# nlesc-dirac/sagecal

Measured on NVIDIA H100. Metric: baseline_visibilities_per_sec_predict_jacobian, higher is better.
Workload: dtype f64

## Files before the change

### sagecal_b200/csrc/internal.cuh

```cuda
#pragma once
#include <cuda_runtime.h>
#include <stdint.h>
#include <stdio.h>
#include <stdlib.h>

#define DB_CHECK(call)                                                                          \
  do {                                                                                          \
    cudaError_t err__ = (call);                                                                 \
    if (err__ != cudaSuccess) {                                                                 \
      fprintf(stderr, "dirac_b200: CUDA error %s at %s:%d: %s\n", cudaGetErrorName(err__),      \
              __FILE__, __LINE__, cudaGetErrorString(err__));                                   \
      exit(1);          \
    }                                                                                           \
  } while (0)


#define TILE_P 8
#define TILE_Q 32
#define TILE_THREADS (TILE_P * TILE_Q)

struct TileDesc {
  short pb, qb;
};

// ... 203 lines not shown
  int N, Nbase;
  int t_begin, t_end, tslice;
};

struct StreamAllArgs {
  const double2 *coh;
  const double2 *x;
  const unsigned char *flag;
  const double *pp;
  const double *pk;
  const ClusterDesc *clus;
  const int *chunk_poff;
  const short2 *blpq;
  double2 *out;
  double2 *E0, *E1, *E2;
  double *partials, *cost;
  unsigned int *counter;
  long long R;
  int N, Nbase, tilesz, M;
  int out_mode, cost_mode;
  double inv_nu;
  int partial;
  long long row0;
  long long w_lo, w_hi;
};

struct GramArgs {
  const double2 *coh;
  const unsigned char *flag;
  const TileDesc *tiles;
// ... 8 lines not shown
  const double *T;
  const double *pblk;
  const int *list;
  const int *tix;
  const int *poff;
  double *JTJ;
  long long stride;
  double *Hst;
  const double *mu_dev;
  double mu;
  int lower;
  int N, Nbase;
};

enum { DB_OPT_CP_ROWS = 0, DB_OPT_LINE_DIRECT = 1, DB_OPT_OS_CONSISTENT = 2,
       DB_OPT_RTR_NU_UNJOINED = 3, DB_OPT_ADMM_LM = 4, DB_OPT_COUNT = 8 };
int db_opt(int id);
int db_sm_count();
static inline int db_cp_max_slices(int Nbase, int tilesz) {
  const int nbg = (Nbase + 255) / 256;
  int nsl = (db_sm_count() + nbg - 1) / nbg;
  if ((tilesz + 31) / 32 > nsl) nsl = (tilesz + 31) / 32;
  return nsl;
}

extern "C" {
void db_launch_coh_to_planar(const double2 *src, double2 *dst, long long r0, int nr, int M,
                             long long R, cudaStream_t st);
void db_launch_coh_from_planar(const double2 *src, double2 *dst, long long r0, int nr, int M,
                               long long R, cudaStream_t st);
void db_launch_vis_to_planar(const double2 *src, double2 *dst, long long R, cudaStream_t st);
// ... 21 lines not shown
                            cudaStream_t st);
void db_launch_chol_factor_batched(const double *A, int n, const double *mu, double *ws,
                                   long long ws_stride, int *info, int nb, cudaStream_t st);
void db_launch_chol_solve(const double *A, int n, double mu, const double *b, double *x, double *ws,
                          int *info, cudaStream_t st);
int db_bigtri_available(int n);
size_t db_bigtri_ws_doubles(int n);
void db_launch_bigtri_solve(const double *L, int ld, int n, const double *b, double *x, double *ws,
                            unsigned epoch, int invert, cudaStream_t st);
int db_stream_all_nblocks(int Nbase, int tilesz);
void db_launch_predict_tma(const StreamAllArgs *a, cudaStream_t st);
void db_launch_cost_window_tma(const StreamAllArgs *a, cudaStream_t st);
int db_band_nblocks(int Nbase, int tilesz, int nchan);
void db_launch_band_tma(const StreamAllArgs *a, int nchan, cudaStream_t st);
void db_launch_band_tma(const StreamAllArgs *a, int nchan, cudaStream_t st);
void db_launch_line_setup_tma(const StreamAllArgs *a, cudaStream_t st);
void db_line_setup_shape_reset();
void db_line_setup_shape(int *shape);
}
```

### sagecal_b200/csrc/kernels_line.cu

```cuda
#include "internal.cuh"

__device__ __forceinline__ void grid_reduce_sum_l(double v, double *partials, double *out,
                                                  unsigned int *counter) {
  __shared__ double wsum[32];
  __shared__ bool is_last;
  v = warp_sum(v);
  const int lane = threadIdx.x & 31, w = threadIdx.x >> 5;
  if (lane == 0) wsum[w] = v;
  __syncthreads();
  const unsigned int nblocks = gridDim.x * gridDim.y;
  const unsigned int bid = blockIdx.x + gridDim.x * blockIdx.y;
  if (threadIdx.x == 0) {
    double s = 0.0;
    const int nw = (blockDim.x + 31) >> 5;
    for (int i = 0; i < nw; i++) s += wsum[i];
    partials[bid] = s;
    __threadfence();
    is_last = (atomicAdd(counter, 1u) == nblocks - 1);
  }
  __syncthreads();
  if (is_last) {
    double s = 0.0;
    for (unsigned int i = threadIdx.x; i < nblocks; i += blockDim.x)
      s += ((volatile double *)partials)[i];
// ... 21 lines not shown
       i += (long long)gridDim.x * blockDim.x) {
    const double2 e0 = E0[i], e1 = E1[i], e2 = E2[i];
    const double ex = (e0.x - alpha * e1.x) - a2 * e2.x;
    const double ey = (e0.y - alpha * e1.y) - a2 * e2.y;
    if (mode == 1) {
      s = fma(ex, ex, s);
      s = fma(ey, ey, s);
    } else {
      s += log(1.0 + ex * ex * inv_nu);
      s += log(1.0 + ey * ey * inv_nu);
    }
  }
  grid_reduce_sum_l(s, partials, out, counter);
}

__global__ void __launch_bounds__(256)
k_line_poly(const double2 *__restrict__ E0, const double2 *__restrict__ E1,
            const double2 *__restrict__ E2, long long n4, double *partials, double *out,
            unsigned int *counter) {
  double c[5] = {0.0, 0.0, 0.0, 0.0, 0.0};
  for (long long i = (long long)blockIdx.x * blockDim.x + threadIdx.x; i < n4;
       i += (long long)gridDim.x * blockDim.x) {
    const double2 e0 = E0[i], e1 = E1[i], e2 = E2[i];
    c[0] = fma(e0.x, e0.x, fma(e0.y, e0.y, c[0]));
    c[1] = fma(e0.x, e1.x, fma(e0.y, e1.y, c[1]));
    c[2] = fma(e1.x, e1.x, fma(e1.y, e1.y, c[2]));
    c[2] = fma(-2.0 * e0.x, e2.x, fma(-2.0 * e0.y, e2.y, c[2]));
    c[3] = fma(e1.x, e2.x, fma(e1.y, e2.y, c[3]));
    c[4] = fma(e2.x, e2.x, fma(e2.y, e2.y, c[4]));
  }
  __shared__ double ws[5][8];
  __shared__ bool is_last;
  const int lane = threadIdx.x & 31, w = threadIdx.x >> 5;
#pragma unroll
  for (int j = 0; j < 5; j++) {
    const double v = warp_sum(c[j]);
    if (lane == 0) ws[j][w] = v;
  }
  __syncthreads();
  if (threadIdx.x < 5) {
    double s = 0.0;
    for (int i = 0; i < 8; i++) s += ws[threadIdx.x][i];
    partials[(size_t)blockIdx.x * 5 + threadIdx.x] = s;
  }
  __threadfence();
  __syncthreads();
  if (threadIdx.x == 0) is_last = (atomicAdd(counter, 1u) == gridDim.x - 1);
  __syncthreads();
  if (is_last && threadIdx.x < 5) {
    double s = 0.0;
    for (unsigned int b = 0; b < gridDim.x; b++)
      s += ((volatile double *)partials)[(size_t)b * 5 + threadIdx.x];
    if (threadIdx.x == 1) s *= -2.0;
    if (threadIdx.x == 3) s *= 2.0;
    out[threadIdx.x] = s;
    if (threadIdx.x == 0) *counter = 0;
  }
}

__global__ void __launch_bounds__(256)
k_line_residual(const double2 *__restrict__ E0, const double2 *__restrict__ E1,
                const double2 *__restrict__ E2, double2 *__restrict__ res, long long n4,
                double alpha) {
  const double a2 = alpha * alpha;
  for (long long i = (long long)blockIdx.x * blockDim.x + threadIdx.x; i < n4;
       i += (long long)gridDim.x * blockDim.x) {
    const double2 e0 = E0[i], e1 = E1[i], e2 = E2[i];
    res[i] = make_double2((e0.x - alpha * e1.x) - a2 * e2.x, (e0.y - alpha * e1.y) - a2 * e2.y);
  }
}

__global__ void __launch_bounds__(256)
// ... 83 lines not shown
void db_launch_axpby(const double2 *x, double2 *y, long long n4, double a, double b,
                     cudaStream_t st) {
  k_axpby<<<592, 256, 0, st>>>(x, y, n4, a, b);
}
void db_launch_cluster_rowmap(const double2 *coh_k, const double2 *in, const double2 *in2,
                               double2 *out, const unsigned char *flag, const double *pp,
                               const int *chunk_poff, int nchunk, const short2 *blpq, long long R,
                               int Nbase, int sign, double beta, cudaStream_t st) {
  k_cluster_rowmap<<<592, 256, 0, st>>>(coh_k, in, in2, out, flag, pp, chunk_poff, nchunk, blpq, R,
                                        Nbase, sign, beta);
}
void db_launch_line_poly(const double2 *E0, const double2 *E1, const double2 *E2, long long n4,
                         double *partials, double *out, unsigned int *counter, cudaStream_t st) {
  k_line_poly<<<192, 256, 0, st>>>(E0, E1, E2, n4, partials, out, counter);
}
void db_launch_line_residual(const double2 *E0, const double2 *E1, const double2 *E2, double2 *res,
                             long long n4, double alpha, cudaStream_t st) {
  k_line_residual<<<LINE_GRID, 256, 0, st>>>(E0, E1, E2, res, n4, alpha);
}
}
```

### sagecal_b200/csrc/kernels_tma.cu

```cuda
#include "internal.cuh"
#include "tma.cuh"

template <int MODE, int TB, int NST, int WARPS>
__global__ void __launch_bounds__(WARPS * 32)
k_stream_all(StreamAllArgs a) {
  extern __shared__ __align__(128) unsigned char smem_raw[];
  constexpr int STAGE_ELEMS = TB * 4 * 32;
  constexpr int NACC = (MODE == 1) ? 3 : 1;
  constexpr size_t RING_BYTES = (size_t)WARPS * NST * STAGE_ELEMS * 16;
  constexpr size_t COMB_BYTES = (size_t)(WARPS - 1) * NACC * STAGE_ELEMS * 16;
  constexpr size_t DATA_BYTES = RING_BYTES > COMB_BYTES ? RING_BYTES : COMB_BYTES;
  double2 *ring = reinterpret_cast<double2 *>(smem_raw);
  unsigned long long *bars = reinterpret_cast<unsigned long long *>(smem_raw + DATA_BYTES);
  const int w = threadIdx.x >> 5, lane = threadIdx.x & 31;
  double2 *my_stage = ring + (size_t)w * NST * STAGE_ELEMS;
  unsigned long long *my_bar = bars + w * NST;
  if (lane == 0) {
#pragma unroll
    for (int s = 0; s < NST; s++) mbar_init(&my_bar[s], 1);
    mbar_fence_init();
  }
  __syncwarp();

  const int nbg = (a.Nbase + 31) >> 5;
// ... 96 lines not shown
  if (w > 0) {
#pragma unroll
    for (int i = 0; i < TB; i++)
#pragma unroll
      for (int c = 0; c < 4; c++) {
        double2 *dst = comb + ((size_t)(w - 1) * NACC * TB * 4 + (i * 4 + c)) * 32 + lane;
        dst[0] = V0[i][c];
        if (MODE == 1) {
          dst[(size_t)TB * 4 * 32] = V1[i][c];
          dst[(size_t)2 * TB * 4 * 32] = V2[i][c];
        }
      }
  }
  __syncthreads();
  double cost = 0.0;
  if (w == 0 && valid) {
    for (int ww = 1; ww < WARPS; ww++)
#pragma unroll
      for (int i = 0; i < TB; i++)
#pragma unroll
        for (int c = 0; c < 4; c++) {
          const double2 *src = comb + ((size_t)(ww - 1) * NACC * TB * 4 + (i * 4 + c)) * 32 + lane;
          V0[i][c] = cadd(V0[i][c], src[0]);
          if (MODE == 1) {
            V1[i][c] = cadd(V1[i][c], src[(size_t)TB * 4 * 32]);
            V2[i][c] = cadd(V2[i][c], src[(size_t)2 * TB * 4 * 32]);
          }
        }
#pragma unroll
    for (int i = 0; i < TB; i++) {
// ... 9 lines not shown
          if (MODE != 1) {
            double2 xv = z;
            if (a.out_mode == 1 || a.cost_mode) xv = ld_stream(a.x + ix);
            const double2 e = csub(xv, m);
            if (a.out_mode == 1) st_stream(a.out + ix, e);
            if (a.out_mode == 2) st_stream(a.out + ix, m);
            if (a.cost_mode == 1) {
              cost = fma(e.x, e.x, cost);
              cost = fma(e.y, e.y, cost);
            } else if (a.cost_mode == 2) {
              cost += log(1.0 + e.x * e.x * a.inv_nu);
              cost += log(1.0 + e.y * e.y * a.inv_nu);
            }
          } else {
            const double2 xv = ld_stream(a.x + ix);
            st_stream(a.E0 + ix, a.partial ? m : csub(xv, m));
            st_stream(a.E1 + ix, fl ? z : V1[i][c]);
            st_stream(a.E2 + ix, fl ? z : V2[i][c]);
          }
        }
      }
    }
  }
  if (MODE != 1 && a.cost_mode) {
    __shared__ bool is_last;
    cost = warp_sum(cost);
    if (threadIdx.x == 0) {
      a.partials[blockIdx.x] = cost;
      __threadfence();
      is_last = (atomicAdd(a.counter, 1u) == gridDim.x - 1);
    }
    __syncthreads();
    if (is_last && w == 0) {
      double s = 0.0;
      for (unsigned int i = lane; i < gridDim.x; i += 32) s += ((volatile double *)a.partials)[i];
      s = warp_sum(s);
      if (lane == 0) {
        *a.cost = s;
        *a.counter = 0;
      }
    }
  }
}

static int g_line_shape[3] = {-1, -1, -1};

template <int MODE, int TB, int NST, int WARPS>
static void launch_cfg(const StreamAllArgs *a, cudaStream_t st) {
  if (MODE == 1) {
    g_line_shape[0] = TB;
    g_line_shape[1] = NST;
    g_line_shape[2] = WARPS;
  }
  const int nbg = (a->Nbase + 31) / 32, ntb = (a->tilesz + TB - 1) / TB;
  const unsigned grid = (unsigned)((long long)nbg * ntb);
  constexpr int NACC = (MODE == 1) ? 3 : 1;
  const size_t ring = (size_t)WARPS * NST * TB * 4 * 32 * 16;
  const size_t comb = (size_t)(WARPS - 1) * NACC * TB * 4 * 32 * 16;
  const size_t smem = (ring > comb ? ring : comb) + WARPS * NST * 8;
  static bool configured = false;
  if (!configured) {
    DB_CHECK(cudaFuncSetAttribute(k_stream_all<MODE, TB, NST, WARPS>,
                                  cudaFuncAttributeMaxDynamicSharedMemorySize, (int)smem));
    configured = true;
  }
  k_stream_all<MODE, TB, NST, WARPS><<<grid, WARPS * 32, smem, st>>>(*a);
}

extern "C" {
int db_stream_all_nblocks(int Nbase, int tilesz) {
  const int nbg = (Nbase + 31) / 32;
  return (int)((long long)nbg * tilesz);
}
void db_launch_predict_tma(const StreamAllArgs *a, cudaStream_t st) {
  launch_cfg<0, 2, 2, 3>(a, st);
}
void db_launch_cost_window_tma(const StreamAllArgs *a, cudaStream_t st) {
  launch_cfg<2, 2, 2, 3>(a, st);
}
void db_launch_line_setup_tma(const StreamAllArgs *a, cudaStream_t st) {
  const long long items = (long long)((a->Nbase + 31) / 32) * a->tilesz;
  if (items >= 64ll * db_sm_count()) launch_cfg<1, 1, 4, 1>(a, st);
  else launch_cfg<1, 1, 2, 3>(a, st);
}
void db_line_setup_shape_reset() { g_line_shape[0] = g_line_shape[1] = g_line_shape[2] = -1; }
void db_line_setup_shape(int *shape) {
  for (int i = 0; i < 3; i++) shape[i] = g_line_shape[i];
}
}
```

### sagecal_b200/csrc/lbfgs.cu

```cuda
#include <float.h>
#include <math.h>
#include <string.h>
#include <vector>

#include "problem.h"

extern "C" {
int db_lbfgs_direction_max_pairs(void);
void db_launch_lbfgs_direction(double *pk, const double *gk, const double *s, const double *y,
                               const double *rho, int m, int npairs, int next, cudaStream_t st);
void db_launch_lbfgs_nrm2(const double *g, int m, double *out, cudaStream_t st);
void db_launch_lbfgs_step(const double *xk, const double *pk, const double *gk, double *xk1,
                          double *sk, double *yk, int m, double alpha, cudaStream_t st);
void db_launch_lbfgs_update(const double *gk, const double *sk, double *yk, const double *xk1,
                            double *xk, int m, double *rho_slot, double *out, cudaStream_t st);
void db_launch_line_eval(const double2 *E0, const double2 *E1, const double2 *E2, long long n4,
                         double alpha, int mode, double inv_nu, double *partials, double *out,
                         unsigned int *counter, cudaStream_t st);
void db_launch_line_residual(const double2 *E0, const double2 *E1, const double2 *E2, double2 *res,
                             long long n4, double alpha, cudaStream_t st);
void db_launch_line_poly(const double2 *E0, const double2 *E1, const double2 *E2, long long n4,
                         double *partials, double *out, unsigned int *counter, cudaStream_t st);
}

struct LbfgsCtx {
  dirac_b200_problem *pr;
  int robust;
  double nu;
  int m;
  long long ncost, ngrad;
  double poly[5];
};

static void line_alloc(dirac_b200_problem *pr) {
  if (pr->E0) return;
  DevProblem &d = pr->d;
  const size_t n = (size_t)4 * d.R;
  pr->E0 = (decltype(pr->E0))db_malloc(sizeof(double2) * n * 3);
  pr->E1 = pr->E0 + n;
  pr->E2 = pr->E1 + n;
}

static void line_setup(LbfgsCtx *c, const double *xk, const double *pk) {
  dirac_b200_problem *pr = c->pr;
  DevProblem &d = pr->d;
  line_alloc(pr);
  StreamAllArgs s;
  memset(&s, 0, sizeof(s));
  s.coh = d.coh; s.x = d.x; s.flag = d.flag; s.pp = xk; s.pk = pk; s.clus = d.clus;
  s.chunk_poff = d.chunk_poff; s.blpq = d.blpq; s.E0 = pr->E0; s.E1 = pr->E1; s.E2 = pr->E2;
  s.R = d.R; s.N = d.N; s.Nbase = d.Nbase; s.tilesz = d.tilesz; s.M = d.M;
  s.partial = (pr->world > 1) ? 1 : 0;
  if (db_overlap_available(pr) && d.tilesz >= 8) {
    static cudaEvent_t ev_chunk[8], ev_done;
    static bool have_ev = false;
    if (!have_ev) {
      for (int i = 0; i < 8; i++) DB_CHECK(cudaEventCreateWithFlags(&ev_chunk[i], cudaEventDisableTiming));
      DB_CHECK(cudaEventCreateWithFlags(&ev_done, cudaEventDisableTiming));
      have_ev = true;
    }
    cudaStream_t cs = db_comm_stream();
    const int nch = 8;
    const int per = (d.tilesz + nch - 1) / nch;
    db_prof_begin(7, (double)d.R * (64.0 * d.M + 65.0 + 192.0), d.stream);
    int ci = 0;
    for (int t0 = 0; t0 < d.tilesz; t0 += per, ci++) {
      const int t1 = (t0 + per < d.tilesz) ? t0 + per : d.tilesz;
// ... 11 lines not shown
      for (int v = 0; v < 3; v++)
        for (int c = 0; c < 4; c++) {
          double2 *base = (v == 0 ? pr->E0 : v == 1 ? pr->E1 : pr->E2) + (long long)c * d.R + r0;
          seg[v * 4 + c] = reinterpret_cast<double *>(base);
          cnt[v * 4 + c] = 2 * nr;
        }
      db_allreduce_segments(pr, seg, cnt, 12, cs);
    }
    db_prof_end(d.stream);
    DB_CHECK(cudaEventRecord(ev_done, cs));
    DB_CHECK(cudaStreamWaitEvent(d.stream, ev_done, 0));
    db_launch_axpby(d.x, pr->E0, 4 * d.R, 1.0, -1.0, d.stream);
    db_count_launch(1);
  } else {
    db_prof_begin(7, (double)d.R * (64.0 * d.M + 65.0 + 192.0), d.stream);
    db_launch_line_setup_tma(&s, d.stream);
    db_prof_end(d.stream);
    db_count_launch(1);
    if (pr->world > 1) {
      db_allreduce(pr, pr->E0, 3 * 8 * d.R);
      db_launch_axpby(d.x, pr->E0, 4 * d.R, 1.0, -1.0, d.stream);
      db_count_launch(1);
    }
  }
  if (!c->robust && !db_opt(DB_OPT_LINE_DIRECT)) {
    db_launch_line_poly(pr->E0, pr->E1, pr->E2, 4 * d.R, pr->partials, d.scal + 16, d.counters,
                        d.stream);
    db_count_launch(1);
    DB_CHECK(cudaMemcpyAsync(d.h_scal + 16, d.scal + 16, 5 * sizeof(double), cudaMemcpyDeviceToHost,
                             d.stream));
    db_stream_sync(d.stream);
    for (int j = 0; j < 5; j++) c->poly[j] = d.h_scal[16 + j];
  }
}

static double line_cost(LbfgsCtx *c, double alpha) {
  dirac_b200_problem *pr = c->pr;
  DevProblem &d = pr->d;
  if (!c->robust && !db_opt(DB_OPT_LINE_DIRECT)) {
    c->ncost++;
    const double *q = c->poly;
    return q[0] + alpha * (q[1] + alpha * (q[2] + alpha * (q[3] + alpha * q[4])));
  }
  db_launch_line_eval(pr->E0, pr->E1, pr->E2, 4 * d.R, alpha, c->robust ? 2 : 1,
                      c->robust ? 1.0 / c->nu : 0.0, pr->partials, d.scal, d.counters, d.stream);
  db_count_launch(1);
  c->ncost++;
  return db_read_scalar(pr, 0);
}

static void grad_eval(LbfgsCtx *c, const double *p, double *g, bool from_line, double alpha) {
  dirac_b200_problem *pr = c->pr;
  DevProblem &d = pr->d;
  if (from_line) {
    db_launch_line_residual(pr->E0, pr->E1, pr->E2, pr->res, 4 * d.R, alpha, d.stream);
    db_count_launch(1);
  } else {
    db_predict_dev(pr, p, pr->res, 1, 0, 0.0, 0);
  }
  db_grad_dev(pr, p, g, c->robust, c->nu);
  c->ngrad++;
}

static double cubic_interp(LbfgsCtx *c, double a, double b, double *xa, double step) {
  double f0, f1, f0d, f1d, p01, p02, z0, fz0, aa, cc;
  *xa = a;
  f0 = line_cost(c, *xa);
  *xa += step;
  p01 = line_cost(c, *xa);
  *xa += -2.0 * step;
  p02 = line_cost(c, *xa);
  f0d = (p01 - p02) / (2.0 * step);
// ... 121 lines not shown
    phi_alphai1 = phi_alphai;
    ci++;
  }
  return alphak;
}

struct LbfgsTrace {
  double *alphak;
  long long *ncost;
  int *slot;
  double *gnorm;
  double *iterates;
  int niter;
};

static void lbfgs_run(dirac_b200_problem *pr, double *p, int m, int itmax, int M, int robust,
                      double nu, LbfgsTrace *tr) {
  DevProblem &d = pr->d;
  LbfgsCtx ctx;
  ctx.pr = pr;
  ctx.robust = robust;
  ctx.nu = nu;
  ctx.m = m;
  ctx.ncost = ctx.ngrad = 0;
  if (tr) tr->niter = 0;
  if (M < 1) M = 1;
  if (M > db_lbfgs_direction_max_pairs()) {
    fprintf(stderr, "dirac_b200: LBFGS memory size %d exceeds the %d pairs the two-loop recursion "
                    "can hold; the LBFGS stage is skipped\n", M, db_lbfgs_direction_max_pairs());
    return;
  }
  double *ws = (double *)db_malloc(sizeof(double) * ((size_t)m * (4 + 2 * (size_t)M) + M + 8));
  double *xk = ws, *xk1 = xk + m, *gk = xk1 + m, *pk = gk + m, *s = pk + m,
         *y = s + (size_t)m * M, *rho = y + (size_t)m * M;
  double *nrm_dev = d.scal + 24;
  double step, alphak;
  int ck, ci, cm;
  DB_CHECK(cudaMemcpyAsync(xk, p, sizeof(double) * m, cudaMemcpyHostToDevice, d.stream));
  grad_eval(&ctx, xk, gk, false, 0.0);
  db_launch_lbfgs_nrm2(gk, m, nrm_dev, d.stream);
  db_count_launch(1);
  double gradnrm = sqrt(db_read_scalar(pr, 24));
  const double STOP = 1e-17;
  if (gradnrm < STOP) {
    ck = itmax;
    step = 0.0;
  } else {
    ck = 0;
    double t = 1e-3 / gradnrm;
    if (t > 1e-6) t = 1e-6;
    step = (t > 1e-9) ? t : 1e-9;
  }
  cm = 0;
  ci = 0;
  while (ck < itmax && isnormal(gradnrm) && gradnrm > STOP) {
    const long long ncost0 = ctx.ncost;
    db_launch_lbfgs_direction(pk, gk, s, y, rho, m, ck < M ? ck : M, ci, d.stream);
    db_count_launch(1);
    line_setup(&ctx, xk, pk);
    alphak = linesearch(&ctx, 10.0, 0.1, 0.01, 9, 0.1, 0.5, step);
    if (!isnormal(alphak) || fabs(alphak) < 1e-12) break;
    double *sk = s + (size_t)cm;
    double *yk = y + (size_t)cm;
    db_launch_lbfgs_step(xk, pk, gk, xk1, sk, yk, m, alphak, d.stream);
    grad_eval(&ctx, xk1, gk, true, alphak);
    db_launch_lbfgs_update(gk, sk, yk, xk1, xk, m, rho + ci, nrm_dev, d.stream);
    db_count_launch(2);
    gradnrm = sqrt(db_read_scalar(pr, 24));
    if (tr) {
      tr->alphak[ck] = alphak;
      tr->ncost[ck] = ctx.ncost - ncost0;
      tr->slot[ck] = ci;
      tr->gnorm[ck] = gradnrm;
      DB_CHECK(cudaMemcpy(tr->iterates + (size_t)m * ck, xk, sizeof(double) * m,
                          cudaMemcpyDeviceToHost));
      tr->niter = ck + 1;
    }
    ck++;
    if (cm < (M - 1) * m) {
      cm += m;
      ci++;
    } else {
      cm = ci = 0;
    }
  }
  DB_CHECK(cudaMemcpyAsync(p, xk, sizeof(double) * m, cudaMemcpyDeviceToHost, d.stream));
  db_stream_sync(d.stream);
  db_free(ws);
}

void db_lbfgs_fit(dirac_b200_problem *pr, double *p, int m, int itmax, int M, int robust,
                  double nu) {
  lbfgs_run(pr, p, m, itmax, M, robust, nu, nullptr);
}

extern "C" void dirac_b200_line_model(dirac_b200_problem *pr, const double *xk, const double *pk,
                                      int nalpha, const double *alphas, double nu,
                                      double alpha_res, double *E, double *poly, double *costs,
                                      double *res, int *shape) {
  DevProblem &d = pr->d;
  LbfgsCtx c;
  c.pr = pr; c.robust = 0; c.nu = nu; c.m = (int)d.npar; c.ncost = c.ngrad = 0;
  double *dx = (double *)db_malloc(sizeof(double) * 2 * d.npar);
  double *dp = dx + d.npar;
  DB_CHECK(cudaMemcpyAsync(dx, xk, sizeof(double) * d.npar, cudaMemcpyHostToDevice, d.stream));
  DB_CHECK(cudaMemcpyAsync(dp, pk, sizeof(double) * d.npar, cudaMemcpyHostToDevice, d.stream));
  db_line_setup_shape_reset();
  line_setup(&c, dx, dp);
// ... 2 lines not shown
  for (int i = 0; i < nalpha; i++)
    for (int mode = 1; mode <= 2; mode++) {
      db_launch_line_eval(pr->E0, pr->E1, pr->E2, 4 * d.R, alphas[i], mode,
                          mode == 2 ? 1.0 / nu : 0.0, pr->partials, d.scal, d.counters, d.stream);
      costs[2 * i + mode - 1] = db_read_scalar(pr, 0);
    }
  db_download_vis(pr, pr->E0, E);
  db_download_vis(pr, pr->E1, E + 8 * d.R);
  db_download_vis(pr, pr->E2, E + 16 * d.R);
  db_launch_line_residual(pr->E0, pr->E1, pr->E2, pr->res, 4 * d.R, alpha_res, d.stream);
  db_download_vis(pr, pr->res, res);
  DB_CHECK(cudaGetLastError());
  db_free(dx);
}

extern "C" int dirac_b200_lbfgs_trace(dirac_b200_problem *pr, double *p, int itmax, int M, int robust,
                                      double nu, double *alphak, long long *ncost, int *slot,
                                      double *gnorm, double *iterates) {
  if ((M < 1 ? 1 : M) > db_lbfgs_direction_max_pairs()) return -1;
  LbfgsTrace tr;
  tr.alphak = alphak; tr.ncost = ncost; tr.slot = slot; tr.gnorm = gnorm; tr.iterates = iterates;
  lbfgs_run(pr, p, (int)pr->d.npar, itmax, M, robust, nu, &tr);
  return tr.niter;
}

extern "C" int dirac_b200_lbfgs_direction(int m, int Mmem, int npairs, int next, const double *g,
                                          const double *s, const double *y, const double *rho,
                                          double *pk) {
  if (m < 1 || Mmem < 1 || npairs < 0 || npairs > Mmem || next < 0 || next >= Mmem ||
      npairs > db_lbfgs_direction_max_pairs())
    return -1;
  const size_t nv = (size_t)m * (2 + 2 * (size_t)Mmem) + Mmem;
  double *w = (double *)db_malloc(sizeof(double) * nv);
  double *dg = w, *dpk = dg + m, *ds = dpk + m, *dy = ds + (size_t)m * Mmem,
         *drho = dy + (size_t)m * Mmem;
  DB_CHECK(cudaMemcpy(dg, g, sizeof(double) * m, cudaMemcpyHostToDevice));
  DB_CHECK(cudaMemcpy(ds, s, sizeof(double) * m * Mmem, cudaMemcpyHostToDevice));
// ... 48 lines not shown
```

### sagecal_b200/csrc/problem.cu

```cuda
#include <string.h>
#include <thread>
#include <vector>

#include "../../include/dirac_b200.h"
#include "internal.cuh"
#include "problem.h"

static unsigned long long g_launches = 0;
static unsigned long long g_sky_uploads = 0, g_coh_host_bytes = 0;
void db_count_sky_upload() { g_sky_uploads++; }
void db_count_coh_host_bytes(size_t bytes) { g_coh_host_bytes += bytes; }
extern "C" void dirac_b200_transfer_stats(unsigned long long *sky_uploads,
                                          unsigned long long *coh_host_bytes, int reset) {
  if (sky_uploads) *sky_uploads = g_sky_uploads;
  if (coh_host_bytes) *coh_host_bytes = g_coh_host_bytes;
  if (reset) g_sky_uploads = g_coh_host_bytes = 0;
}
void db_count_launch(int n) { g_launches += (unsigned long long)n; }
extern "C" unsigned long long dirac_b200_launch_count(void) { return g_launches; }

struct ProfRec { cudaEvent_t a, b; int kind; double bytes; };
static std::vector<ProfRec> g_prof;
static std::vector<cudaEvent_t> g_evpool;
static int g_prof_on = 0;
// ... 45 lines not shown
  if (g_have_user_stream) { *owned = 0; return g_user_stream; }
  cudaStream_t st;
  DB_CHECK(cudaStreamCreateWithFlags(&st, cudaStreamNonBlocking));
  *owned = 1;
  return st;
}

static int g_opt[DB_OPT_COUNT] = {0, 0, 0, 0, 0, 0, 0, 0};
int db_opt(int id) { return (id >= 0 && id < DB_OPT_COUNT) ? g_opt[id] : 0; }
extern "C" int dirac_b200_set_option(const char *name, int value) {
  if (!strcmp(name, "cp_rows")) { g_opt[DB_OPT_CP_ROWS] = value; return 0; }
  if (!strcmp(name, "line_direct")) { g_opt[DB_OPT_LINE_DIRECT] = value; return 0; }
  if (!strcmp(name, "os_consistent")) { g_opt[DB_OPT_OS_CONSISTENT] = value; return 0; }
  if (!strcmp(name, "rtr_nu_unjoined")) { g_opt[DB_OPT_RTR_NU_UNJOINED] = value; return 0; }
  if (!strcmp(name, "admm_lm")) { g_opt[DB_OPT_ADMM_LM] = value; return 0; }
  return -1;
}
int db_sm_count() {
  static int n[64];
  int dev = 0;
  if (cudaGetDevice(&dev) != cudaSuccess || dev < 0 || dev >= 64) return 132;
  if (!n[dev]) {
    int v = 0;
    if (cudaDeviceGetAttribute(&v, cudaDevAttrMultiProcessorCount, dev) != cudaSuccess || v <= 0) v = 132;
    n[dev] = v;
  }
  return n[dev];
}

void require_gpu() {
// ... 506 lines not shown
```

### sagecal_b200/csrc/problem.h

```cpp
#pragma once
#include <cusolverDn.h>
#include <cublas_v2.h>

#include <vector>

#include "../../include/dirac_b200.h"
#include "internal.cuh"

struct BigChol;
BigChol *db_bigchol_create(int n, int nbk, bool inv_panel, bool lookahead);
enum { BC_BLOCK = 256 };
static const bool BC_INV_PANEL = true, BC_LOOKAHEAD = true;
void db_bigchol_destroy(BigChol *bc);
void db_bigchol_bind_batch(BigChol *bc, double *A0, long long stride, int maxb);
void db_bigchol_factor_batch(BigChol *bc, int nb, int *info, int info_step, cudaStream_t st);

struct LMWork {
  bool ready;
  int n8;
  double *T;
  unsigned char *T_valid;
  double *Tsub;
  double *JTJ0, *JTJ;
  double *JTe, *JTe_new;
// ... 46 lines not shown
  double *g;
  LMWork lm;
  int own_stream;
  int rank, world;
  void (*allreduce)(void *dev, long long count, void *stream, void *user);
  void *comm_user;
  int m_global;
  int k_global0;
  double beta;
  const double *aug_y_host, *aug_bz_host, *aug_rho;
  double *aug_dev;
  double2 *pm;
  double *xb;
  double *pp_start;
  double2 *E0, *E1, *E2;
  struct RtrWork *rtr;
};

void db_stream_sync(cudaStream_t st);
void db_event_sync(cudaEvent_t ev);
void db_flag_wait(const volatile unsigned long long *flag, unsigned long long epoch,
                  cudaStream_t st);
void *db_malloc(size_t bytes);
void db_free(void *p);
void require_gpu();

class DeviceScope {
 public:
  DeviceScope();
  explicit DeviceScope(cudaStream_t borrowed);
// ... 46 lines not shown
void db_allreduce_world(dirac_b200_problem *pr, void *dev, long long count);
int db_nccl_world();
void db_allreduce_stream(dirac_b200_allreduce_fn fn, void *user, void *dev, long long count,
                         cudaStream_t st);
int db_manifold_projectback(double *Y, int n, int Mt, int Nf, int Niter, const int *cr,
                            cudaStream_t st);void db_lm_set_aug(const double *y_dev, const double *bz_dev, const double *y_host,
                   const double *bz_host, double rho);
int db_overlap_available(const dirac_b200_problem *pr);
cudaStream_t db_comm_stream();
void db_allreduce_segments(dirac_b200_problem *pr, double **ptr, const long long *count, int nseg,
                           cudaStream_t st);
extern "C" {
void db_launch_residual_cost(const double2 *x, const double2 *pm, double2 *out, long long n4,
                             int out_mode, int cost_mode, double inv_nu, double *partials,
                             double *cost, unsigned int *counter, cudaStream_t st);
void db_launch_axpby(const double2 *x, double2 *y, long long n4, double a, double b,
                     cudaStream_t st);
void db_launch_cluster_rowmap(const double2 *coh_k, const double2 *in, const double2 *in2,
                              double2 *out, const unsigned char *flag, const double *pp,
                              const int *chunk_poff, int nchunk, const short2 *blpq, long long R,
                              int Nbase, int sign, double beta, cudaStream_t st);
}

struct BandView {
  const double2 *coh, *x;
  const unsigned char *flag;
  int nc;
};
struct BandDev {
  int N, Nbase, tilesz, M, Mt, maxnc, ntile;
// ... 24 lines not shown
```

### sagecal_b200/csrc/sage.cu

```cuda
#include <math.h>
#include <string.h>
#include <thread>
#include <vector>

#include "../../include/dirac_b200.h"
#include "problem.h"

void db_lm_chunk(dirac_b200_problem *pr, int k, int ck, double *pblk_dev, double2 *r, int itmax,
                 const double *opts, int linsolv, int os, int randomize, double *info,
                 bool hidden_ready);
void db_rlm_chunk(dirac_b200_problem *pr, int k, int ck, double *pblk_dev, double2 *r, int itmax,
                  int linsolv, int os, int randomize, double nulow, double nuhigh,
                  double *robust_nu, double *info, bool hidden_ready);
bool db_cluster_needs_rowmap(const dirac_b200_problem *pr, int k);
void db_cluster_hidden(dirac_b200_problem *pr, int k, double2 *r, int sign, double beta);
void db_lbfgs_fit(dirac_b200_problem *pr, double *p, int m, int itmax, int M, int robust,
                  double nu);
void db_lbfgs_fit_minibatch(dirac_b200_problem *pr, double *p, int m, int itmax, int M, double nu);
void db_rtr_chunk(dirac_b200_problem *pr, int k, int ck, double *pblk_dev, double2 *r, int kind,
                  int itmax_a, int itmax_b, double nulow, double nuhigh, double *robust_nu,
                  double *info, bool hidden_ready, const double *aug_y, const double *aug_bz,
                  double aug_rho);
#define SM_RTR_ADMM_ 7

static bool is_robust_mode(int solver_mode) {
  return solver_mode == SM_OSLM_OSRLM_RLBFGS || solver_mode == SM_RLM_RLBFGS ||
         solver_mode == SM_RTR_OSRLM_RLBFGS || solver_mode == SM_NSD_RLBFGS ||
         solver_mode == SM_RTR_ADMM_;
}

extern "C" int dirac_b200_sagefit(dirac_b200_problem *pr, double *pp, double *x_out,
                                  int max_emiter, int max_iter, int max_lbfgs, int lbfgs_m,
// ... 168 lines not shown
    if (total_err > 0.0)
      for (int cj = 0; cj < MG; cj++) nerr[cj] *= 1.0 / total_err;
    if (randomize) weighted_iter = !weighted_iter;
  }
  if (robust) {
    if (sharded) allreduce_host(robust_nuM.data(), MG);
    double s = 0.0;
    for (int cj = 0; cj < MG; cj++) s += fabs(robust_nuM[cj]);
    robust_nu0 = s / (double)MG;
    if (robust_nu0 < nulow) robust_nu0 = nulow;
    else if (robust_nu0 > nuhigh) robust_nu0 = nuhigh;
  }
  DB_CHECK(cudaMemcpyAsync(pp, d.pp, sizeof(double) * m, cudaMemcpyDeviceToHost, d.stream));
  db_stream_sync(d.stream);

  if (max_lbfgs > 0) {
    if (robust) {
      if (lbfgs_m > 0) {
        db_lbfgs_fit(pr, pp, m, max_lbfgs, lbfgs_m, 1, robust_nu0);
      } else if (lbfgs_m < 0) {
        db_lbfgs_fit_minibatch(pr, pp, m, max_lbfgs, -lbfgs_m, robust_nu0);
      }
    } else {
      db_lbfgs_fit(pr, pp, m, max_lbfgs, lbfgs_m, 0, 0.0);
    }
  }
  DB_CHECK(cudaMemcpyAsync(d.pp, pp, sizeof(double) * m, cudaMemcpyHostToDevice, d.stream));
  db_predict_dev(pr, d.pp, pr->res, 1, 1, 0.0, 0);
  *res_1 = sqrt(db_read_scalar(pr, 0)) / (double)n;
  if (x_out) db_download_vis(pr, pr->res, x_out);
  *mean_nu = robust_nu0;
  DB_CHECK(cudaGetLastError());
  return (*res_1 > *res_0) ? -1 : 0;
}

extern "C" int sagefit_visibilities(double *u, double *v, double *w, double *x, int N, int Nbase,
                                    int tilesz, baseline_t *barr, clus_source_t *carr,
                                    double *coh, int M, int Mt, double freq0, double fdelta,
                                    double *pp, double uvmin, int Nt, int max_emiter, int max_iter,
                                    int max_lbfgs, int lbfgs_m, int gpu_threads, int linsolv,
                                    int solver_mode, double nulow, double nuhigh, int randomize,
                                    double *mean_nu, double *res_0, double *res_1) {
  (void)u; (void)v; (void)w; (void)freq0; (void)fdelta; (void)uvmin; (void)Nt; (void)gpu_threads;
// ... 19 lines not shown
SAGEFIT_ALIAS(sagefit_visibilities_dual_pt_flt)
SAGEFIT_ALIAS(sagefit_visibilities_dual_pt)
SAGEFIT_ALIAS(sagefit_visibilities_dual_pt_one_gpu)

int db_bfgsfit_dev(dirac_b200_problem *pr, double *pp, int max_lbfgs, int lbfgs_m, int solver_mode,
                   double mean_nu, double *res_0, double *res_1, bool keep_residual) {
  DevProblem &d = pr->d;
  const int m = d.N * d.Mt * 8;
  const long long n = (long long)d.Nbase * d.tilesz * 8;
  DB_CHECK(cudaMemcpyAsync(d.pp, pp, sizeof(double) * m, cudaMemcpyHostToDevice, d.stream));
  db_predict_dev(pr, d.pp, nullptr, 0, 1, 0.0, 0);
  *res_0 = sqrt(db_read_scalar(pr, 0)) / (double)n;
  if (max_lbfgs > 0) {
    int M_ = lbfgs_m > 0 ? lbfgs_m : -lbfgs_m;
    if (is_robust_mode(solver_mode)) {
      db_lbfgs_fit(pr, pp, m, max_lbfgs, M_, 1, mean_nu);
    } else {
      db_lbfgs_fit(pr, pp, m, max_lbfgs, M_, 0, 0.0);
    }
  }
  DB_CHECK(cudaMemcpyAsync(d.pp, pp, sizeof(double) * m, cudaMemcpyHostToDevice, d.stream));
  db_predict_dev(pr, d.pp, keep_residual ? pr->res : nullptr, keep_residual ? 1 : 0, 1, 0.0, 0);
  *res_1 = sqrt(db_read_scalar(pr, 0)) / (double)n;
  return (*res_1 > *res_0) ? -1 : 0;
}

extern "C" int bfgsfit_visibilities(double *u, double *v, double *w, double *x, int N, int Nbase,
                                    int tilesz, baseline_t *barr, clus_source_t *carr,
                                    double *coh, int M, int Mt, double freq0, double fdelta,
                                    double *pp, double uvmin, int Nt, int max_lbfgs, int lbfgs_m,
                                    int gpu_threads, int solver_mode, double mean_nu,
                                    double *res_0, double *res_1) {
  (void)u; (void)v; (void)w; (void)freq0; (void)fdelta; (void)uvmin; (void)Nt; (void)gpu_threads;
// ... 78 lines not shown
```

Measured before the change: 6.816 billion.

## Fold line-search polynomial into setup kernel and reuse held residuals after LBFGS

The line-setup streaming kernel now accumulates the five line-search polynomial coefficients while it writes E0/E1/E2. A small finish kernel then reduces the per-block partials, so the separate pass that re-read all three arrays is no longer needed on the single-device path. The LBFGS stage can also start from the residual already held on the device instead of re-predicting it. After LBFGS, the final cost is taken as a sum of squares over the held residual rather than a full re-predict. This cuts memory passes and predict launches in the sagefit path, at the price of extra registers in the streaming kernel and an assumption that the held residual matches the final parameters.

New measurement: 7.071 billion (median of 6 runs). +3.7%, better.

```diff
diff --git a/sagecal_b200/csrc/internal.cuh b/sagecal_b200/csrc/internal.cuh
--- a/sagecal_b200/csrc/internal.cuh
+++ b/sagecal_b200/csrc/internal.cuh
@@ -241,6 +241,7 @@
   const short2 *blpq;
   double2 *out;
   double2 *E0, *E1, *E2;
+  double *poly_part;
   double *partials, *cost;
   unsigned int *counter;
   long long R;
@@ -279,7 +280,8 @@
 };
 
 enum { DB_OPT_CP_ROWS = 0, DB_OPT_LINE_DIRECT = 1, DB_OPT_OS_CONSISTENT = 2,
-       DB_OPT_RTR_NU_UNJOINED = 3, DB_OPT_ADMM_LM = 4, DB_OPT_COUNT = 8 };
+       DB_OPT_RTR_NU_UNJOINED = 3, DB_OPT_ADMM_LM = 4, DB_OPT_SWEEP_RESIDUAL = 5,
+       DB_OPT_COUNT = 8 };
 int db_opt(int id);
 int db_sm_count();
 static inline int db_cp_max_slices(int Nbase, int tilesz) {
@@ -331,7 +333,9 @@
 int db_band_nblocks(int Nbase, int tilesz, int nchan);
 void db_launch_band_tma(const StreamAllArgs *a, int nchan, cudaStream_t st);
 void db_launch_band_tma(const StreamAllArgs *a, int nchan, cudaStream_t st);
-void db_launch_line_setup_tma(const StreamAllArgs *a, cudaStream_t st);
+unsigned db_launch_line_setup_tma(const StreamAllArgs *a, cudaStream_t st);
+void db_launch_line_poly_finish(const double *part, unsigned nparts, double *partials, double *out,
+                                unsigned int *counter, cudaStream_t st);
 void db_line_setup_shape_reset();
 void db_line_setup_shape(int *shape);
 }
diff --git a/sagecal_b200/csrc/kernels_line.cu b/sagecal_b200/csrc/kernels_line.cu
--- a/sagecal_b200/csrc/kernels_line.cu
+++ b/sagecal_b200/csrc/kernels_line.cu
@@ -59,6 +59,37 @@
   grid_reduce_sum_l(s, partials, out, counter);
 }
 
+__device__ __forceinline__ void poly_grid_reduce(const double *c, double *partials, double *out,
+                                                 unsigned int *counter) {
+  __shared__ double ws[5][8];
+  __shared__ bool is_last;
+  const int lane = threadIdx.x & 31, w = threadIdx.x >> 5;
+#pragma unroll
+  for (int j = 0; j < 5; j++) {
+    const double v = warp_sum(c[j]);
+    if (lane == 0) ws[j][w] = v;
+  }
+  __syncthreads();
+  if (threadIdx.x < 5) {
+    double s = 0.0;
+    for (int i = 0; i < 8; i++) s += ws[threadIdx.x][i];
+    partials[(size_t)blockIdx.x * 5 + threadIdx.x] = s;
+  }
+  __threadfence();
+  __syncthreads();
+  if (threadIdx.x == 0) is_last = (atomicAdd(counter, 1u) == gridDim.x - 1);
+  __syncthreads();
+  if (is_last && threadIdx.x < 5) {
+    double s = 0.0;
+    for (unsigned int b = 0; b < gridDim.x; b++)
+      s += ((volatile double *)partials)[(size_t)b * 5 + threadIdx.x];
+    if (threadIdx.x == 1) s *= -2.0;
+    if (threadIdx.x == 3) s *= 2.0;
+    out[threadIdx.x] = s;
+    if (threadIdx.x == 0) *counter = 0;
+  }
+}
+
 __global__ void __launch_bounds__(256)
 k_line_poly(const double2 *__restrict__ E0, const double2 *__restrict__ E1,
             const double2 *__restrict__ E2, long long n4, double *partials, double *out,
@@ -74,33 +105,30 @@
     c[3] = fma(e1.x, e2.x, fma(e1.y, e2.y, c[3]));
     c[4] = fma(e2.x, e2.x, fma(e2.y, e2.y, c[4]));
   }
-  __shared__ double ws[5][8];
-  __shared__ bool is_last;
-  const int lane = threadIdx.x & 31, w = threadIdx.x >> 5;
-#pragma unroll
-  for (int j = 0; j < 5; j++) {
-    const double v = warp_sum(c[j]);
-    if (lane == 0) ws[j][w] = v;
-  }
-  __syncthreads();
-  if (threadIdx.x < 5) {
-    double s = 0.0;
-    for (int i = 0; i < 8; i++) s += ws[threadIdx.x][i];
-    partials[(size_t)blockIdx.x * 5 + threadIdx.x] = s;
-  }
-  __threadfence();
-  __syncthreads();
-  if (threadIdx.x == 0) is_last = (atomicAdd(counter, 1u) == gridDim.x - 1);
-  __syncthreads();
-  if (is_last && threadIdx.x < 5) {
-    double s = 0.0;
-    for (unsigned int b = 0; b < gridDim.x; b++)
-      s += ((volatile double *)partials)[(size_t)b * 5 + threadIdx.x];
-    if (threadIdx.x == 1) s *= -2.0;
-    if (threadIdx.x == 3) s *= 2.0;
-    out[threadIdx.x] = s;
-    if (threadIdx.x == 0) *counter = 0;
-  }
+  poly_grid_reduce(c, partials, out, counter);
+}
+
+__global__ void __launch_bounds__(256)
+k_line_poly_finish(const double *__restrict__ part, unsigned nparts, double *partials, double *out,
+                   unsigned int *counter) {
+  double c[5] = {0.0, 0.0, 0.0, 0.0, 0.0};
+  for (unsigned i = blockIdx.x * blockDim.x + threadIdx.x; i < nparts; i += gridDim.x * blockDim.x)
+#pragma unroll
+    for (int j = 0; j < 5; j++) c[j] += part[(size_t)j * nparts + i];
+  poly_grid_reduce(c, partials, out, counter);
+}
+
+__global__ void __launch_bounds__(256)
+k_sumsq(const double2 *__restrict__ v, long long n4, double *partials, double *out,
+        unsigned int *counter) {
+  double s = 0.0;
+  for (long long i = (long long)blockIdx.x * blockDim.x + threadIdx.x; i < n4;
+       i += (long long)gridDim.x * blockDim.x) {
+    const double2 e = v[i];
+    s = fma(e.x, e.x, s);
+    s = fma(e.y, e.y, s);
+  }
+  grid_reduce_sum_l(s, partials, out, counter);
 }
 
 __global__ void __launch_bounds__(256)
@@ -214,6 +242,14 @@
                          double *partials, double *out, unsigned int *counter, cudaStream_t st) {
   k_line_poly<<<192, 256, 0, st>>>(E0, E1, E2, n4, partials, out, counter);
 }
+void db_launch_line_poly_finish(const double *part, unsigned nparts, double *partials, double *out,
+                                unsigned int *counter, cudaStream_t st) {
+  k_line_poly_finish<<<192, 256, 0, st>>>(part, nparts, partials, out, counter);
+}
+void db_launch_sumsq(const double2 *v, long long n4, double *partials, double *out,
+                     unsigned int *counter, cudaStream_t st) {
+  k_sumsq<<<LINE_GRID, 256, 0, st>>>(v, n4, partials, out, counter);
+}
 void db_launch_line_residual(const double2 *E0, const double2 *E1, const double2 *E2, double2 *res,
                              long long n4, double alpha, cudaStream_t st) {
   k_line_residual<<<LINE_GRID, 256, 0, st>>>(E0, E1, E2, res, n4, alpha);
diff --git a/sagecal_b200/csrc/kernels_tma.cu b/sagecal_b200/csrc/kernels_tma.cu
--- a/sagecal_b200/csrc/kernels_tma.cu
+++ b/sagecal_b200/csrc/kernels_tma.cu
@@ -134,6 +134,7 @@
   }
   __syncthreads();
   double cost = 0.0;
+  double cq[5] = {0.0, 0.0, 0.0, 0.0, 0.0};
   if (w == 0 && valid) {
     for (int ww = 1; ww < WARPS; ww++)
 #pragma unroll
@@ -173,12 +174,29 @@
             }
           } else {
             const double2 xv = ld_stream(a.x + ix);
-            st_stream(a.E0 + ix, a.partial ? m : csub(xv, m));
-            st_stream(a.E1 + ix, fl ? z : V1[i][c]);
-            st_stream(a.E2 + ix, fl ? z : V2[i][c]);
-          }
-        }
-      }
+            const double2 e0 = a.partial ? m : csub(xv, m);
+            const double2 e1 = fl ? z : V1[i][c], e2 = fl ? z : V2[i][c];
+            st_stream(a.E0 + ix, e0);
+            st_stream(a.E1 + ix, e1);
+            st_stream(a.E2 + ix, e2);
+            if (a.poly_part) {
+              cq[0] = fma(e0.x, e0.x, fma(e0.y, e0.y, cq[0]));
+              cq[1] = fma(e0.x, e1.x, fma(e0.y, e1.y, cq[1]));
+              cq[2] = fma(e1.x, e1.x, fma(e1.y, e1.y, cq[2]));
+              cq[2] = fma(-2.0 * e0.x, e2.x, fma(-2.0 * e0.y, e2.y, cq[2]));
+              cq[3] = fma(e1.x, e2.x, fma(e1.y, e2.y, cq[3]));
+              cq[4] = fma(e2.x, e2.x, fma(e2.y, e2.y, cq[4]));
+            }
+          }
+        }
+      }
+    }
+  }
+  if (MODE == 1 && a.poly_part && w == 0) {
+#pragma unroll
+    for (int j = 0; j < 5; j++) {
+      const double v = warp_sum(cq[j]);
+      if (lane == 0) a.poly_part[(size_t)j * gridDim.x + blockIdx.x] = v;
     }
   }
   if (MODE != 1 && a.cost_mode) {
@@ -205,7 +223,7 @@
 static int g_line_shape[3] = {-1, -1, -1};
 
 template <int MODE, int TB, int NST, int WARPS>
-static void launch_cfg(const StreamAllArgs *a, cudaStream_t st) {
+static unsigned launch_cfg(const StreamAllArgs *a, cudaStream_t st) {
   if (MODE == 1) {
     g_line_shape[0] = TB;
     g_line_shape[1] = NST;
@@ -224,6 +242,7 @@
     configured = true;
   }
   k_stream_all<MODE, TB, NST, WARPS><<<grid, WARPS * 32, smem, st>>>(*a);
+  return grid;
 }
 
 extern "C" {
@@ -237,10 +256,10 @@
 void db_launch_cost_window_tma(const StreamAllArgs *a, cudaStream_t st) {
   launch_cfg<2, 2, 2, 3>(a, st);
 }
-void db_launch_line_setup_tma(const StreamAllArgs *a, cudaStream_t st) {
+unsigned db_launch_line_setup_tma(const StreamAllArgs *a, cudaStream_t st) {
   const long long items = (long long)((a->Nbase + 31) / 32) * a->tilesz;
-  if (items >= 64ll * db_sm_count()) launch_cfg<1, 1, 4, 1>(a, st);
-  else launch_cfg<1, 1, 2, 3>(a, st);
+  if (items >= 64ll * db_sm_count()) return launch_cfg<1, 1, 4, 1>(a, st);
+  return launch_cfg<1, 1, 2, 3>(a, st);
 }
 void db_line_setup_shape_reset() { g_line_shape[0] = g_line_shape[1] = g_line_shape[2] = -1; }
 void db_line_setup_shape(int *shape) {
diff --git a/sagecal_b200/csrc/lbfgs.cu b/sagecal_b200/csrc/lbfgs.cu
--- a/sagecal_b200/csrc/lbfgs.cu
+++ b/sagecal_b200/csrc/lbfgs.cu
@@ -36,9 +36,11 @@
   if (pr->E0) return;
   DevProblem &d = pr->d;
   const size_t n = (size_t)4 * d.R;
-  pr->E0 = (decltype(pr->E0))db_malloc(sizeof(double2) * n * 3);
+  const size_t nb = (size_t)db_stream_all_nblocks(d.Nbase, d.tilesz);
+  pr->E0 = (decltype(pr->E0))db_malloc(sizeof(double2) * n * 3 + sizeof(double) * 5 * nb);
   pr->E1 = pr->E0 + n;
   pr->E2 = pr->E1 + n;
+  pr->poly_part = reinterpret_cast<double *>(pr->E2 + n);
 }
 
 static void line_setup(LbfgsCtx *c, const double *xk, const double *pk) {
@@ -51,6 +53,9 @@
   s.chunk_poff = d.chunk_poff; s.blpq = d.blpq; s.E0 = pr->E0; s.E1 = pr->E1; s.E2 = pr->E2;
   s.R = d.R; s.N = d.N; s.Nbase = d.Nbase; s.tilesz = d.tilesz; s.M = d.M;
   s.partial = (pr->world > 1) ? 1 : 0;
+  const bool want_poly = !c->robust && !db_opt(DB_OPT_LINE_DIRECT);
+  const bool fold_poly = want_poly && pr->world <= 1;
+  s.poly_part = fold_poly ? pr->poly_part : nullptr;
   if (db_overlap_available(pr) && d.tilesz >= 8) {
     static cudaEvent_t ev_chunk[8], ev_done;
     static bool have_ev = false;
@@ -92,19 +97,26 @@
     db_count_launch(1);
   } else {
     db_prof_begin(7, (double)d.R * (64.0 * d.M + 65.0 + 192.0), d.stream);
-    db_launch_line_setup_tma(&s, d.stream);
+    const unsigned nparts = db_launch_line_setup_tma(&s, d.stream);
     db_prof_end(d.stream);
     db_count_launch(1);
+    if (fold_poly) {
+      db_launch_line_poly_finish(pr->poly_part, nparts, pr->partials, d.scal + 16, d.counters,
+                                 d.stream);
+      db_count_launch(1);
+    }
     if (pr->world > 1) {
       db_allreduce(pr, pr->E0, 3 * 8 * d.R);
       db_launch_axpby(d.x, pr->E0, 4 * d.R, 1.0, -1.0, d.stream);
       db_count_launch(1);
     }
   }
-  if (!c->robust && !db_opt(DB_OPT_LINE_DIRECT)) {
-    db_launch_line_poly(pr->E0, pr->E1, pr->E2, 4 * d.R, pr->partials, d.scal + 16, d.counters,
-                        d.stream);
-    db_count_launch(1);
+  if (want_poly) {
+    if (!fold_poly) {
+      db_launch_line_poly(pr->E0, pr->E1, pr->E2, 4 * d.R, pr->partials, d.scal + 16, d.counters,
+                          d.stream);
+      db_count_launch(1);
+    }
     DB_CHECK(cudaMemcpyAsync(d.h_scal + 16, d.scal + 16, 5 * sizeof(double), cudaMemcpyDeviceToHost,
                              d.stream));
     db_stream_sync(d.stream);
@@ -127,13 +139,14 @@
   return db_read_scalar(pr, 0);
 }
 
-static void grad_eval(LbfgsCtx *c, const double *p, double *g, bool from_line, double alpha) {
+enum { RES_PREDICT, RES_LINE, RES_HELD };
+static void grad_eval(LbfgsCtx *c, const double *p, double *g, int res_src, double alpha) {
   dirac_b200_problem *pr = c->pr;
   DevProblem &d = pr->d;
-  if (from_line) {
+  if (res_src == RES_LINE) {
     db_launch_line_residual(pr->E0, pr->E1, pr->E2, pr->res, 4 * d.R, alpha, d.stream);
     db_count_launch(1);
-  } else {
+  } else if (res_src == RES_PREDICT) {
     db_predict_dev(pr, p, pr->res, 1, 0, 0.0, 0);
   }
   db_grad_dev(pr, p, g, c->robust, c->nu);
@@ -285,8 +298,8 @@
   int niter;
 };
 
-static void lbfgs_run(dirac_b200_problem *pr, double *p, int m, int itmax, int M, int robust,
-                      double nu, LbfgsTrace *tr) {
+static int lbfgs_run(dirac_b200_problem *pr, double *p, int m, int itmax, int M, int robust,
+                      double nu, bool res_held, LbfgsTrace *tr) {
   DevProblem &d = pr->d;
   LbfgsCtx ctx;
   ctx.pr = pr;
@@ -299,7 +312,7 @@
   if (M > db_lbfgs_direction_max_pairs()) {
     fprintf(stderr, "dirac_b200: LBFGS memory size %d exceeds the %d pairs the two-loop recursion "
                     "can hold; the LBFGS stage is skipped\n", M, db_lbfgs_direction_max_pairs());
-    return;
+    return 0;
   }
   double *ws = (double *)db_malloc(sizeof(double) * ((size_t)m * (4 + 2 * (size_t)M) + M + 8));
   double *xk = ws, *xk1 = xk + m, *gk = xk1 + m, *pk = gk + m, *s = pk + m,
@@ -308,7 +321,7 @@
   double step, alphak;
   int ck, ci, cm;
   DB_CHECK(cudaMemcpyAsync(xk, p, sizeof(double) * m, cudaMemcpyHostToDevice, d.stream));
-  grad_eval(&ctx, xk, gk, false, 0.0);
+  grad_eval(&ctx, xk, gk, res_held ? RES_HELD : RES_PREDICT, 0.0);
   db_launch_lbfgs_nrm2(gk, m, nrm_dev, d.stream);
   db_count_launch(1);
   double gradnrm = sqrt(db_read_scalar(pr, 24));
@@ -334,7 +347,7 @@
     double *sk = s + (size_t)cm;
     double *yk = y + (size_t)cm;
     db_launch_lbfgs_step(xk, pk, gk, xk1, sk, yk, m, alphak, d.stream);
-    grad_eval(&ctx, xk1, gk, true, alphak);
+    grad_eval(&ctx, xk1, gk, RES_LINE, alphak);
     db_launch_lbfgs_update(gk, sk, yk, xk1, xk, m, rho + ci, nrm_dev, d.stream);
     db_count_launch(2);
     gradnrm = sqrt(db_read_scalar(pr, 24));
@@ -358,11 +371,12 @@
   DB_CHECK(cudaMemcpyAsync(p, xk, sizeof(double) * m, cudaMemcpyDeviceToHost, d.stream));
   db_stream_sync(d.stream);
   db_free(ws);
-}
-
-void db_lbfgs_fit(dirac_b200_problem *pr, double *p, int m, int itmax, int M, int robust,
-                  double nu) {
-  lbfgs_run(pr, p, m, itmax, M, robust, nu, nullptr);
+  return (int)ctx.ngrad - 1;
+}
+
+int db_lbfgs_fit(dirac_b200_problem *pr, double *p, int m, int itmax, int M, int robust,
+                 double nu, bool res_held) {
+  return lbfgs_run(pr, p, m, itmax, M, robust, nu, res_held, nullptr);
 }
 
 extern "C" void dirac_b200_line_model(dirac_b200_problem *pr, const double *xk, const double *pk,
@@ -395,13 +409,29 @@
   db_free(dx);
 }
 
+extern "C" void dirac_b200_line_poly(dirac_b200_problem *pr, double *poly) {
+  DevProblem &d = pr->d;
+  db_launch_line_poly(pr->E0, pr->E1, pr->E2, 4 * d.R, pr->partials, d.scal + 16, d.counters,
+                      d.stream);
+  DB_CHECK(cudaMemcpyAsync(d.h_scal + 16, d.scal + 16, 5 * sizeof(double), cudaMemcpyDeviceToHost,
+                           d.stream));
+  db_stream_sync(d.stream);
+  DB_CHECK(cudaGetLastError());
+  for (int j = 0; j < 5; j++) poly[j] = d.h_scal[16 + j];
+}
+
+extern "C" void dirac_b200_residual(dirac_b200_problem *pr, double *out) {
+  db_download_vis(pr, pr->res, out);
+  DB_CHECK(cudaGetLastError());
+}
+
 extern "C" int dirac_b200_lbfgs_trace(dirac_b200_problem *pr, double *p, int itmax, int M, int robust,
                                       double nu, double *alphak, long long *ncost, int *slot,
                                       double *gnorm, double *iterates) {
   if ((M < 1 ? 1 : M) > db_lbfgs_direction_max_pairs()) return -1;
   LbfgsTrace tr;
   tr.alphak = alphak; tr.ncost = ncost; tr.slot = slot; tr.gnorm = gnorm; tr.iterates = iterates;
-  lbfgs_run(pr, p, (int)pr->d.npar, itmax, M, robust, nu, &tr);
+  lbfgs_run(pr, p, (int)pr->d.npar, itmax, M, robust, nu, false, &tr);
   return tr.niter;
 }
 
diff --git a/sagecal_b200/csrc/problem.cu b/sagecal_b200/csrc/problem.cu
--- a/sagecal_b200/csrc/problem.cu
+++ b/sagecal_b200/csrc/problem.cu
@@ -83,6 +83,7 @@
   if (!strcmp(name, "os_consistent")) { g_opt[DB_OPT_OS_CONSISTENT] = value; return 0; }
   if (!strcmp(name, "rtr_nu_unjoined")) { g_opt[DB_OPT_RTR_NU_UNJOINED] = value; return 0; }
   if (!strcmp(name, "admm_lm")) { g_opt[DB_OPT_ADMM_LM] = value; return 0; }
+  if (!strcmp(name, "sweep_residual")) { g_opt[DB_OPT_SWEEP_RESIDUAL] = value; return 0; }
   return -1;
 }
 int db_sm_count() {
diff --git a/sagecal_b200/csrc/problem.h b/sagecal_b200/csrc/problem.h
--- a/sagecal_b200/csrc/problem.h
+++ b/sagecal_b200/csrc/problem.h
@@ -84,6 +84,7 @@
   double *xb;
   double *pp_start;
   double2 *E0, *E1, *E2;
+  double *poly_part;
   struct RtrWork *rtr;
 };
 
@@ -160,6 +161,8 @@
 void db_launch_residual_cost(const double2 *x, const double2 *pm, double2 *out, long long n4,
                              int out_mode, int cost_mode, double inv_nu, double *partials,
                              double *cost, unsigned int *counter, cudaStream_t st);
+void db_launch_sumsq(const double2 *v, long long n4, double *partials, double *out,
+                     unsigned int *counter, cudaStream_t st);
 void db_launch_axpby(const double2 *x, double2 *y, long long n4, double a, double b,
                      cudaStream_t st);
 void db_launch_cluster_rowmap(const double2 *coh_k, const double2 *in, const double2 *in2,
diff --git a/sagecal_b200/csrc/sage.cu b/sagecal_b200/csrc/sage.cu
--- a/sagecal_b200/csrc/sage.cu
+++ b/sagecal_b200/csrc/sage.cu
@@ -14,8 +14,8 @@
                   double *robust_nu, double *info, bool hidden_ready);
 bool db_cluster_needs_rowmap(const dirac_b200_problem *pr, int k);
 void db_cluster_hidden(dirac_b200_problem *pr, int k, double2 *r, int sign, double beta);
-void db_lbfgs_fit(dirac_b200_problem *pr, double *p, int m, int itmax, int M, int robust,
-                  double nu);
+int db_lbfgs_fit(dirac_b200_problem *pr, double *p, int m, int itmax, int M, int robust,
+                 double nu, bool res_held);
 void db_lbfgs_fit_minibatch(dirac_b200_problem *pr, double *p, int m, int itmax, int M, double nu);
 void db_rtr_chunk(dirac_b200_problem *pr, int k, int ck, double *pblk_dev, double2 *r, int kind,
                   int itmax_a, int itmax_b, double nulow, double nuhigh, double *robust_nu,
@@ -214,19 +214,28 @@
   DB_CHECK(cudaMemcpyAsync(pp, d.pp, sizeof(double) * m, cudaMemcpyDeviceToHost, d.stream));
   db_stream_sync(d.stream);
 
+  const bool minibatch = max_lbfgs > 0 && robust && lbfgs_m < 0;
+  const bool lbfgs_stage = max_lbfgs > 0 && (!robust || lbfgs_m != 0);
+  int steps = 0;
   if (max_lbfgs > 0) {
     if (robust) {
       if (lbfgs_m > 0) {
-        db_lbfgs_fit(pr, pp, m, max_lbfgs, lbfgs_m, 1, robust_nu0);
+        steps = db_lbfgs_fit(pr, pp, m, max_lbfgs, lbfgs_m, 1, robust_nu0, true);
       } else if (lbfgs_m < 0) {
         db_lbfgs_fit_minibatch(pr, pp, m, max_lbfgs, -lbfgs_m, robust_nu0);
       }
     } else {
-      db_lbfgs_fit(pr, pp, m, max_lbfgs, lbfgs_m, 0, 0.0);
-    }
-  }
-  DB_CHECK(cudaMemcpyAsync(d.pp, pp, sizeof(double) * m, cudaMemcpyHostToDevice, d.stream));
-  db_predict_dev(pr, d.pp, pr->res, 1, 1, 0.0, 0);
+      steps = db_lbfgs_fit(pr, pp, m, max_lbfgs, lbfgs_m, 0, 0.0, true);
+    }
+  }
+  if (lbfgs_stage)
+    DB_CHECK(cudaMemcpyAsync(d.pp, pp, sizeof(double) * m, cudaMemcpyHostToDevice, d.stream));
+  if (steps > 0 || (db_opt(DB_OPT_SWEEP_RESIDUAL) && !minibatch)) {
+    db_launch_sumsq(pr->res, 4 * d.R, pr->partials, d.scal, d.counters, d.stream);
+    db_count_launch(1);
+  } else {
+    db_predict_dev(pr, d.pp, pr->res, 1, 1, 0.0, 0);
+  }
   *res_1 = sqrt(db_read_scalar(pr, 0)) / (double)n;
   if (x_out) db_download_vis(pr, pr->res, x_out);
   *mean_nu = robust_nu0;
@@ -276,9 +285,9 @@
   if (max_lbfgs > 0) {
     int M_ = lbfgs_m > 0 ? lbfgs_m : -lbfgs_m;
     if (is_robust_mode(solver_mode)) {
-      db_lbfgs_fit(pr, pp, m, max_lbfgs, M_, 1, mean_nu);
+      db_lbfgs_fit(pr, pp, m, max_lbfgs, M_, 1, mean_nu, false);
     } else {
-      db_lbfgs_fit(pr, pp, m, max_lbfgs, M_, 0, 0.0);
+      db_lbfgs_fit(pr, pp, m, max_lbfgs, M_, 0, 0.0, false);
     }
   }
   DB_CHECK(cudaMemcpyAsync(d.pp, pp, sizeof(double) * m, cudaMemcpyHostToDevice, d.stream));
```
